# joyfang1106/MRLA

Measured on AMD Instinct MI355X. Metric: images/sec fwd+bwd resnet50_mrlal b=256, higher is better.
Workload: dtype bf16

## Files before the change

### mrla_amd/csrc/conv1x1.hip

```cpp
#include <algorithm>

#include "mrla_device.h"
#include "mrla_kernels.h"

namespace mrla {

typedef __bf16 bf16x8 __attribute__((ext_vector_type(8)));
typedef float f32x16 __attribute__((ext_vector_type(16)));

constexpr int kOutRowB = 64 * 2 + 16;
constexpr int kOutTileB = 32 * kOutRowB;

__device__ __forceinline__ int acc_channel(int reg, int h) { return (reg & 3) + 8 * (reg >> 2) + 4 * h; }

template <int KS, bool MOM, int NW>
__global__ __launch_bounds__(NW * kWave) void conv1x1_fwd_kernel(
    const bf16_t* __restrict__ X, const bf16_t* __restrict__ W, bf16_t* __restrict__ Y, float* __restrict__ part,
    int M, int N, int NS, int WN, int rows_total) {
  constexpr int K = KS * 16;
  constexpr int ROWB = K * 2 + 16;
  constexpr int KC = KS < 16 ? KS : 16;
  constexpr int NCH = KS / KC;
  constexpr bool DB = KS <= 16;
  extern __shared__ __align__(16) unsigned char smem_raw[];
  const int lane = threadIdx.x & (kWave - 1), wave = threadIdx.x / kWave;
  const int r = lane & 31, h = lane >> 5;
  const int WM = NW / WN, wn = wave % WN, wm = wave / WN;
  const int n_slice0 = blockIdx.y * NS;
  unsigned char* otile = smem_raw + (size_t)NS * ROWB + (size_t)wave * kOutTileB;

  {
    constexpr int PPR = K / 8;
    const u32x4* wsrc = reinterpret_cast<const u32x4*>(W + (size_t)n_slice0 * K);
    for (int i = threadIdx.x; i < NS * PPR; i += NW * kWave) {
      const int row = i / PPR, pc = i - row * PPR;
      *reinterpret_cast<u32x4*>(smem_raw + (size_t)row * ROWB + pc * 16) = wsrc[i];
    }
  }
  __syncthreads();

  float s1[2][16], s2[2][16], pv[2][16];
#pragma unroll
  for (int t = 0; t < 2; ++t)
#pragma unroll
    for (int i = 0; i < 16; ++i) { s1[t][i] = 0.f; s2[t][i] = 0.f; pv[t][i] = 0.f; }
  bool have_pivot = false;
  int npix = 0;

  const int nblk = (M + 31) / 32;
  const int stride = gridDim.x * WM;
  int blk = blockIdx.x * WM + wm;
  u32x4 xf[KC], xn[DB ? KC : 1];
  auto load_x = [&](u32x4 (&dst)[KC], int b_, int kc) {
    const int row = min(b_ * 32 + r, M - 1);
    const u32x4* xp = reinterpret_cast<const u32x4*>(X + (size_t)row * K + kc * KC * 16 + h * 8);
#pragma unroll
    for (int ks = 0; ks < KC; ++ks) dst[ks] = xp[ks * 2];
  };
  if (blk < nblk) load_x(xf, blk, 0);
  for (; blk < nblk; blk += stride) {
    if constexpr (DB) {
      if (blk + stride < nblk) load_x(reinterpret_cast<u32x4(&)[KC]>(xn), blk + stride, 0);
    }
    const bool live = blk * 32 + r < M;
    npix += min(32, M - blk * 32);
    f32x16 acc[2];
#pragma unroll
    for (int t = 0; t < 2; ++t)
#pragma unroll
      for (int i = 0; i < 16; ++i) acc[t][i] = 0.f;
#pragma unroll 1
    for (int kc = 0; kc < NCH; ++kc) {
      if (kc > 0) load_x(xf, blk, kc);
#pragma unroll
      for (int t = 0; t < 2; ++t) {
        const unsigned char* wrow = smem_raw + (size_t)(wn * 64 + t * 32 + r) * ROWB + kc * KC * 32 + h * 16;
#pragma unroll
        for (int ks = 0; ks < KC; ++ks) {
          const u32x4 wf = *reinterpret_cast<const u32x4*>(wrow + ks * 32);
          acc[t] = __builtin_amdgcn_mfma_f32_32x32x16_bf16(__builtin_bit_cast(bf16x8, wf),
                                                           __builtin_bit_cast(bf16x8, xf[ks]), acc[t], 0, 0, 0);
        }
      }
    }
#pragma unroll
    for (int t = 0; t < 2; ++t) {
      unsigned p[8];
#pragma unroll
      for (int i = 0; i < 8; ++i) {
        typedef bf16_t bf16x2 __attribute__((ext_vector_type(2)));
        bf16x2 pr;
        pr[0] = from_f<bf16_t>(acc[t][2 * i]);
        pr[1] = from_f<bf16_t>(acc[t][2 * i + 1]);
        p[i] = __builtin_bit_cast(unsigned, pr);
      }
      if (MOM) {
#pragma unroll
        for (int i = 0; i < 8; ++i) {
          const float lo = __uint_as_float(p[i] << 16), hi = __uint_as_float(p[i] & 0xffff0000u);
          if (!have_pivot) {
            pv[t][2 * i] = __shfl(lo, h * 32, kWave);
            pv[t][2 * i + 1] = __shfl(hi, h * 32, kWave);
          }
          const float dl = live ? lo - pv[t][2 * i] : 0.f, dh = live ? hi - pv[t][2 * i + 1] : 0.f;
          s1[t][2 * i] += dl;     s2[t][2 * i] = fmaf(dl, dl, s2[t][2 * i]);
          s1[t][2 * i + 1] += dh; s2[t][2 * i + 1] = fmaf(dh, dh, s2[t][2 * i + 1]);
        }
      }
#if defined(__HIP_DEVICE_COMPILE__)
#pragma unroll
      for (int g = 0; g < 2; ++g) {
#pragma unroll
        for (int q = 0; q < 2; ++q) {
          const auto sw = __builtin_amdgcn_permlane32_swap(p[4 * g + q], p[4 * g + 2 + q], false, false);
          p[4 * g + q] = sw[0];
          p[4 * g + 2 + q] = sw[1];
        }
      }
#endif
      unsigned char* orow = otile + r * kOutRowB + (t * 32 + h * 8) * 2;
      *reinterpret_cast<u32x4*>(orow) = (u32x4){p[0], p[1], p[2], p[3]};
      *reinterpret_cast<u32x4*>(orow + 32) = (u32x4){p[4], p[5], p[6], p[7]};
    }
    have_pivot = true;
    {
      const int px = lane >> 3, piece = lane & 7;
      bf16_t* ybase = Y + (size_t)blk * 32 * N + n_slice0 + wn * 64 + piece * 8;
#pragma unroll
      for (int i = 0; i < 4; ++i) {
        const int pr = i * 8 + px;
        const u32x4 v = *reinterpret_cast<const u32x4*>(otile + pr * kOutRowB + piece * 16);
        if (blk * 32 + pr < M) *reinterpret_cast<u32x4*>(ybase + (size_t)pr * N) = v;
      }
    }
    if constexpr (DB) {
#pragma unroll
      for (int ks = 0; ks < KC; ++ks) xf[ks] = xn[ks];
    } else {
      if (blk + stride < nblk) load_x(xf, blk + stride, 0);
    }
  }

  if (MOM) {
    if (blockIdx.x == 0) {
      for (int i = threadIdx.x; i < (rows_total - (int)gridDim.x) * NS * 4; i += NW * kWave) {
        const int row = gridDim.x + i / (NS * 4), j = i % (NS * 4);
        part[((size_t)row * N + n_slice0) * 4 + j] = 0.f;
      }
    }
    __syncthreads();
    float* sums = reinterpret_cast<float*>(smem_raw + (size_t)NS * ROWB);
#pragma unroll
    for (int t = 0; t < 2; ++t)
#pragma unroll
      for (int i = 0; i < 16; ++i) {
        float a = s1[t][i], b = s2[t][i];
#pragma unroll
        for (int off = 16; off > 0; off >>= 1) {
          a += __shfl_xor(a, off, kWave);
          b += __shfl_xor(b, off, kWave);
        }
        if (r == 0) {
          const int ch = wn * 64 + t * 32 + acc_channel(i, h);
          float* rec = sums + ((size_t)wm * NS + ch) * 4;
          rec[0] = a; rec[1] = b; rec[2] = pv[t][i]; rec[3] = (float)npix;
        }
      }
    __syncthreads();
    float* dst = part + ((size_t)blockIdx.x * N + n_slice0) * 4;
    for (int ch = threadIdx.x; ch < NS; ch += NW * kWave) {
      float S1 = 0.f, S2 = 0.f, P = 0.f, n = 0.f;
      for (int v = 0; v < WM; ++v) {
        const float* rec = sums + ((size_t)v * NS + ch) * 4;
        const float a = rec[0], b = rec[1], nv = rec[3];
        if (nv == 0.f) continue;
        if (n == 0.f) P = rec[2];
        const float dlt = rec[2] - P;
        S2 += b + 2.f * dlt * a + nv * dlt * dlt;
        S1 += a + nv * dlt;
        n += nv;
      }
      dst[ch * 4 + 0] = S1; dst[ch * 4 + 1] = S2; dst[ch * 4 + 2] = P; dst[ch * 4 + 3] = n;
    }
  }
}

struct GemmGeo { int NS, WN, WM, NW, gx, gy, rows; size_t lds; };

static bool conv1x1_geo(GemmGeo* g, int M, int K, int N) {
  if (K != 64 && K != 128 && K != 256) return false;
  if (N % 64 || M <= 0) return false;
  const int rowb = K * 2 + 16;
  int ns = std::min(N, 256);
  while (ns > 64 && (N % ns || (ns / 64 != 1 && ns / 64 != 2 && ns / 64 != 4) || (size_t)ns * rowb > 72 * 1024)) ns -= 64;
  if (N % ns) return false;
  g->NS = ns;
  g->WN = ns / 64;
  g->NW = K <= 128 ? 4 : 8;
  if (g->NW < g->WN) g->NW = g->WN;
  g->WM = g->NW / g->WN;
  g->gy = N / ns;
  g->lds = (size_t)ns * rowb + (size_t)g->NW * kOutTileB;
  const int nblk = (M + 31) / 32;
  const int want = std::max(1, (256 * (g->NW == 4 ? 3 : 2)) / g->gy);
  int gx = std::max(1, std::min((nblk + g->WM - 1) / g->WM, want));
  for (int t = gx; t >= std::max(1, gx - gx / 4); --t)
    if (M % t == 0) { gx = t; break; }
  int rows = gx;
  while (rows <= 2 * gx + 64 && M % rows) ++rows;
  if (M % rows) return false;
  g->gx = gx;
  g->rows = rows;
  return true;
}

int conv1x1_rows(int M, int K, int N) {
  const int wide = conv1x1_wide_rows(M, K, N);
  if (wide > 0) return wide;
  GemmGeo g;
  if (conv1x1_geo(&g, M, K, N)) return g.rows;
  return conv1x1_kstream_supported(M, K, N) ? conv1x1_kstream_rows(M, K, N) : MRLA_EUNSUPPORTED;
}

int conv1x1_plan(int M, int K, int N, int add, int* out) {
  if (conv1x1_wide_plan(M, K, N, add, out) == MRLA_OK) return MRLA_OK;
  GemmGeo g;
  if (!add && !conv1x1_geo(&g, M, K, N) && conv1x1_kstream_supported(M, K, N)) {
    out[0] = K / 32; out[1] = conv1x1_kstream_stages(M, K, N); out[2] = 0; out[3] = conv1x1_kstream_rows(M, K, N);
    return MRLA_OK;
  }
  if (add || !conv1x1_geo(&g, M, K, N)) return MRLA_EUNSUPPORTED;
  const int nblk = (M + 31) / 32;
  out[0] = (nblk + g.gx * g.WM - 1) / (g.gx * g.WM);
  out[1] = 2;
  out[2] = g.gx * g.gy;
  out[3] = g.rows;
  return MRLA_OK;
}

int launch_conv1x1_fwd(const void* x, const void* w, void* y, float* part, int M, int K, int N, hipStream_t st) {
  if (conv1x1_wide_rows(M, K, N) > 0) return launch_conv1x1_wide(x, w, nullptr, y, part, M, K, N, st);
  GemmGeo g;
  if (!conv1x1_geo(&g, M, K, N)) {
    if (!conv1x1_kstream_supported(M, K, N)) return MRLA_EUNSUPPORTED;
    return launch_conv1x1_kstream(x, w, y, part, M, K, N, st);
  }
  const dim3 grid(g.gx, g.gy), block(g.NW * kWave);
#define CALL_W(KS, MO, NWV)                                                                                          \
  {                                                                                                                  \
    if (lds_opt_in(reinterpret_cast<const void*>(conv1x1_fwd_kernel<KS, MO, NWV>), g.lds) != hipSuccess)              \
      return MRLA_EHIP;                                                                                              \
    hipLaunchKernelGGL((conv1x1_fwd_kernel<KS, MO, NWV>), grid, block, g.lds, st, (const bf16_t*)x, (const bf16_t*)w, \
                       (bf16_t*)y, part, M, N, g.NS, g.WN, g.rows);                                                  \
  }
#define CALL_M(KS, MO) { if (g.NW == 4) CALL_W(KS, MO, 4) else CALL_W(KS, MO, 8) }
#define CALL(KS) { if (part) CALL_M(KS, true) else CALL_M(KS, false) }
  switch (K) {
    case 64:  CALL(4) break;
    case 128: CALL(8) break;
    case 256: CALL(16) break;
    default: return MRLA_EUNSUPPORTED;
  }
#undef CALL
#undef CALL_M
#undef CALL_W
  return hip_status(hipGetLastError());
}

}
```

Baseline: 8532.

## Accumulate BN moment statistics from LDS output tile in store-lane layout

Moves the per-channel sum and sum-of-squares accumulation out of the MFMA accumulator layout, where each lane held 32 channels, and into the coalesced store loop. There each lane reads the staged output tile and owns 8 channels. This shrinks the moment registers from 96 floats to 24 per lane and shortens the final cross-lane reduction, aiming to cut VGPR pressure and shuffle work. The K=256 path also drops its 4-wave instantiation, so geometries choosing NW=4 there now return unsupported.

```diff
diff --git a/mrla_amd/csrc/conv1x1.hip b/mrla_amd/csrc/conv1x1.hip
--- a/mrla_amd/csrc/conv1x1.hip
+++ b/mrla_amd/csrc/conv1x1.hip
@@ -39,11 +39,9 @@
   }
   __syncthreads();
 
-  float s1[2][16], s2[2][16], pv[2][16];
-#pragma unroll
-  for (int t = 0; t < 2; ++t)
-#pragma unroll
-    for (int i = 0; i < 16; ++i) { s1[t][i] = 0.f; s2[t][i] = 0.f; pv[t][i] = 0.f; }
+  float s1[8], s2[8], pv[8];
+#pragma unroll
+  for (int i = 0; i < 8; ++i) { s1[i] = 0.f; s2[i] = 0.f; pv[i] = 0.f; }
   bool have_pivot = false;
   int npix = 0;
 
@@ -62,7 +60,6 @@
     if constexpr (DB) {
       if (blk + stride < nblk) load_x(reinterpret_cast<u32x4(&)[KC]>(xn), blk + stride, 0);
     }
-    const bool live = blk * 32 + r < M;
     npix += min(32, M - blk * 32);
     f32x16 acc[2];
 #pragma unroll
@@ -94,19 +91,6 @@
         pr[1] = from_f<bf16_t>(acc[t][2 * i + 1]);
         p[i] = __builtin_bit_cast(unsigned, pr);
       }
-      if (MOM) {
-#pragma unroll
-        for (int i = 0; i < 8; ++i) {
-          const float lo = __uint_as_float(p[i] << 16), hi = __uint_as_float(p[i] & 0xffff0000u);
-          if (!have_pivot) {
-            pv[t][2 * i] = __shfl(lo, h * 32, kWave);
-            pv[t][2 * i + 1] = __shfl(hi, h * 32, kWave);
-          }
-          const float dl = live ? lo - pv[t][2 * i] : 0.f, dh = live ? hi - pv[t][2 * i + 1] : 0.f;
-          s1[t][2 * i] += dl;     s2[t][2 * i] = fmaf(dl, dl, s2[t][2 * i]);
-          s1[t][2 * i + 1] += dh; s2[t][2 * i + 1] = fmaf(dh, dh, s2[t][2 * i + 1]);
-        }
-      }
 #if defined(__HIP_DEVICE_COMPILE__)
 #pragma unroll
       for (int g = 0; g < 2; ++g) {
@@ -122,17 +106,32 @@
       *reinterpret_cast<u32x4*>(orow) = (u32x4){p[0], p[1], p[2], p[3]};
       *reinterpret_cast<u32x4*>(orow + 32) = (u32x4){p[4], p[5], p[6], p[7]};
     }
-    have_pivot = true;
     {
       const int px = lane >> 3, piece = lane & 7;
       bf16_t* ybase = Y + (size_t)blk * 32 * N + n_slice0 + wn * 64 + piece * 8;
+      if (MOM && !have_pivot) {
+        const u32x4 p0 = *reinterpret_cast<const u32x4*>(otile + piece * 16);
+#pragma unroll
+        for (int j = 0; j < 4; ++j) { pv[2 * j] = __uint_as_float(p0[j] << 16); pv[2 * j + 1] = __uint_as_float(p0[j] & 0xffff0000u); }
+      }
 #pragma unroll
       for (int i = 0; i < 4; ++i) {
         const int pr = i * 8 + px;
         const u32x4 v = *reinterpret_cast<const u32x4*>(otile + pr * kOutRowB + piece * 16);
-        if (blk * 32 + pr < M) *reinterpret_cast<u32x4*>(ybase + (size_t)pr * N) = v;
-      }
-    }
+        const bool lv = blk * 32 + pr < M;
+        if (lv) *reinterpret_cast<u32x4*>(ybase + (size_t)pr * N) = v;
+        if (MOM) {
+#pragma unroll
+          for (int j = 0; j < 4; ++j) {
+            const float lo = __uint_as_float(v[j] << 16), hi = __uint_as_float(v[j] & 0xffff0000u);
+            const float dl = lv ? lo - pv[2 * j] : 0.f, dh = lv ? hi - pv[2 * j + 1] : 0.f;
+            s1[2 * j] += dl;     s2[2 * j] = fmaf(dl, dl, s2[2 * j]);
+            s1[2 * j + 1] += dh; s2[2 * j + 1] = fmaf(dh, dh, s2[2 * j + 1]);
+          }
+        }
+      }
+    }
+    have_pivot = true;
     if constexpr (DB) {
 #pragma unroll
       for (int ks = 0; ks < KC; ++ks) xf[ks] = xn[ks];
@@ -151,21 +150,19 @@
     __syncthreads();
     float* sums = reinterpret_cast<float*>(smem_raw + (size_t)NS * ROWB);
 #pragma unroll
-    for (int t = 0; t < 2; ++t)
-#pragma unroll
-      for (int i = 0; i < 16; ++i) {
-        float a = s1[t][i], b = s2[t][i];
-#pragma unroll
-        for (int off = 16; off > 0; off >>= 1) {
-          a += __shfl_xor(a, off, kWave);
-          b += __shfl_xor(b, off, kWave);
-        }
-        if (r == 0) {
-          const int ch = wn * 64 + t * 32 + acc_channel(i, h);
-          float* rec = sums + ((size_t)wm * NS + ch) * 4;
-          rec[0] = a; rec[1] = b; rec[2] = pv[t][i]; rec[3] = (float)npix;
-        }
-      }
+    for (int i = 0; i < 8; ++i) {
+      float a = s1[i], b = s2[i];
+#pragma unroll
+      for (int off = 32; off >= 8; off >>= 1) {
+        a += __shfl_xor(a, off, kWave);
+        b += __shfl_xor(b, off, kWave);
+      }
+      if (lane < 8) {
+        const int ch = wn * 64 + lane * 8 + i;
+        float* rec = sums + ((size_t)wm * NS + ch) * 4;
+        rec[0] = a; rec[1] = b; rec[2] = pv[i]; rec[3] = (float)npix;
+      }
+    }
     __syncthreads();
     float* dst = part + ((size_t)blockIdx.x * N + n_slice0) * 4;
     for (int ch = threadIdx.x; ch < NS; ch += NW * kWave) {
@@ -258,7 +255,10 @@
   switch (K) {
     case 64:  CALL(4) break;
     case 128: CALL(8) break;
-    case 256: CALL(16) break;
+    case 256:
+      if (g.NW != 8) return MRLA_EUNSUPPORTED;
+      if (part) CALL_W(16, true, 8) else CALL_W(16, false, 8)
+      break;
     default: return MRLA_EUNSUPPORTED;
   }
 #undef CALL
```

Result: faster. 8715, median of 6 (+2.1%).
